# fabrizio-m/TyPLONK

Hardware: AMD Instinct MI355X
Metric: msm_g1_adds_per_s (higher is better)
Workload: dtype u32; 1 GPU; 2^20-term BLS12-381 G1 MSM (KZG commit of a 2^20-row polynomial), SRS [s^i]G with s=2, 1048579 points; window_bits=20, windows=13, parallelism=single GPU, fixed_base_tables=c=20, 13 tables per rank

## Files before the change

### typlonk_amd/csrc/harness/device_reduce_rows.hip

```cpp
#include "../msm_reduce.hip"

#include <algorithm>

using namespace ty;

namespace {

struct Bufs {
    void* p[8] = {};
    int used = 0;
    hipError_t err = hipSuccess;
    uint32_t* zeros(uint64_t points) {
        void* d = nullptr;
        const size_t bytes = (size_t)std::max<uint64_t>(points, 1) * 192;
        if (err == hipSuccess) err = hipMalloc(&d, bytes);
        if (err == hipSuccess) p[used++] = d;
        if (err == hipSuccess) err = hipMemset(d, 0, bytes);
        return static_cast<uint32_t*>(d);
    }
    ~Bufs() {
        for (int i = 0; i < used; ++i) (void)hipFree(p[i]);
    }
};

bool shape_ok(const RcShape& sh) {
    if (sh.nsets < 1 || sh.nsets > 32 || sh.c1 != sh.cl + sh.ch || sh.c1 > 19) return false;
    if (sh.cl < 6 || sh.ch < 6 || sh.cl > 12 || sh.ch > 12 || sh.lhc > sh.ch || sh.llc > sh.cl) return false;
    if (sh.cl - sh.llc > 7 || sh.ch - sh.lhc > 7) return false;
    for (uint32_t set = 0; set < sh.nsets; ++set) {
        uint32_t nbr, nbc, shift;
        rc_bits(sh, set, &nbr, &nbc, &shift);
        if (nbr > RC_NB || nbc > RC_NB) return false;
    }
    return true;
}

__global__ __launch_bounds__(256) void add_pairs_kernel(const uint32_t* __restrict__ a, const uint32_t* __restrict__ b, uint32_t npairs,
                                                        uint32_t* rows_out, uint32_t* lane_out, uint32_t* slow) {
    __shared__ uint32_t buf[4][3][FQR_POINT_WORDS];
    const uint32_t wave = threadIdx.x >> 6, lane = threadIdx.x & 63u, w = blockIdx.x * 4 + wave;
    if (w >= npairs) return;
    const uint32_t c = lane >> 4, i = lane & 15u;
    buf[wave][0][lane] = fqr_limb_of_words(a + (uint64_t)w * 48 + c * 12, i);
    buf[wave][1][lane] = fqr_limb_of_words(b + (uint64_t)w * 48 + c * 12, i);
    __builtin_amdgcn_fence(__ATOMIC_RELEASE, "wavefront");
    __builtin_amdgcn_wave_barrier();
    __builtin_amdgcn_fence(__ATOMIC_ACQUIRE, "wavefront");
    const bool s = g1_add_rows<RowsDev>(buf[wave][0], buf[wave][1], buf[wave][2]);
    __builtin_amdgcn_fence(__ATOMIC_RELEASE, "wavefront");
    __builtin_amdgcn_wave_barrier();
    __builtin_amdgcn_fence(__ATOMIC_ACQUIRE, "wavefront");
    fqr_store_rows<RowsDev>(rows_out + (uint64_t)w * 48, buf[wave][2][lane]);
    if (lane == 0) {
        slow[w] = s ? 1u : 0u;
        st_xyzz(lane_out, w, g1_add(ld_xyzz(a, w), ld_xyzz(b, w)));
    }
}

}

extern "C" int drr_add_pairs(const uint32_t* a, const uint32_t* b, uint32_t npairs, uint32_t* rows_out, uint32_t* lane_out,
                             uint32_t* slow) {
    if (npairs < 1 || npairs > 4096) return (int)hipErrorInvalidValue;
    Bufs m;
    uint32_t* d_a = m.zeros(npairs);
    uint32_t* d_b = m.zeros(npairs);
    uint32_t* d_r = m.zeros(npairs);
    uint32_t* d_l = m.zeros(npairs);
    uint32_t* d_s = m.zeros((npairs + 47) / 48);
    if (m.err == hipSuccess) m.err = hipMemcpy(d_a, a, (size_t)npairs * 192, hipMemcpyHostToDevice);
    if (m.err == hipSuccess) m.err = hipMemcpy(d_b, b, (size_t)npairs * 192, hipMemcpyHostToDevice);
    if (m.err == hipSuccess) {
        hipLaunchKernelGGL(add_pairs_kernel, dim3((npairs + 3) / 4), dim3(256), 0, 0, d_a, d_b, npairs, d_r, d_l, d_s);
        m.err = hipGetLastError();
    }
    if (m.err == hipSuccess) m.err = hipDeviceSynchronize();
    if (m.err == hipSuccess) m.err = hipMemcpy(rows_out, d_r, (size_t)npairs * 192, hipMemcpyDeviceToHost);
    if (m.err == hipSuccess) m.err = hipMemcpy(lane_out, d_l, (size_t)npairs * 192, hipMemcpyDeviceToHost);
    if (m.err == hipSuccess) m.err = hipMemcpy(slow, d_s, (size_t)npairs * 4, hipMemcpyDeviceToHost);
    return (int)m.err;
}

extern "C" int drr_reduce(int form, const uint32_t* shape, const uint32_t* buckets, uint32_t* planes) {
    RcShape sh;
    sh.nsets = shape[0];
    sh.c1 = shape[1];
    sh.ch = shape[2];
    sh.cl = shape[3];
    sh.lhc = shape[4];
    sh.llc = shape[5];
    sh.top_v = shape[6];
    if ((form != 0 && form != 1) || !shape_ok(sh) || !msm_rows_ok(sh)) return (int)hipErrorInvalidValue;
    const uint64_t nb = (uint64_t)sh.nsets << sh.c1;
    const uint64_t nrow = (uint64_t)sh.nsets << (sh.c1 - sh.llc), ncol = (uint64_t)sh.nsets << (sh.c1 - sh.lhc);
    const uint64_t nplanes = (uint64_t)sh.nsets * 2 * RC_NB;
    Bufs m;
    uint32_t* d_buckets = m.zeros(nb);
    uint32_t* part_b = m.zeros(nrow);
    uint32_t* part_a = m.zeros(ncol);
    uint32_t* sums = m.zeros(((uint64_t)sh.nsets << sh.ch) + ((uint64_t)sh.nsets << sh.cl));
    uint32_t* bitsum = m.zeros(nplanes * 64);
    uint32_t* d_planes = m.zeros(nplanes);
    if (m.err == hipSuccess) m.err = hipMemcpy(d_buckets, buckets, (size_t)nb * 192, hipMemcpyHostToDevice);
    if (m.err == hipSuccess) {
        launch_msm_rc_reduce_form(d_buckets, sh, part_b, part_a, sums, bitsum, d_planes, form == 0, 0);
        m.err = hipGetLastError();
    }
    if (m.err == hipSuccess) m.err = hipDeviceSynchronize();
    if (m.err == hipSuccess) m.err = hipMemcpy(planes, d_planes, (size_t)nplanes * 192, hipMemcpyDeviceToHost);
    return (int)m.err;
}
```

### typlonk_amd/csrc/launch.hpp

```cpp
#pragma once
#include <hip/hip_runtime.h>
#include <stdint.h>
#include "ff.hpp"
#include "msm_plan.hpp"
#include "ntt_args.hpp"

namespace ty {

constexpr int PT_WORDS = 32;
constexpr int MSM_HEAVY_GRID = 1024;

struct QuotientArgs {
    const Fr* wires[3];
    const Fr* z;
    const Fr* sel[5];
    const Fr* sigma[3];
    const Fr* pi;
    const Fr* l0;
    const Fr* w_lo;
    const Fr* bx_hi;
    Fr* out;
    uint64_t n4;
    uint32_t w_h;
    uint32_t k0_is_one;
    Fr alpha, alpha2, beta, gamma;
    Fr k[3];
    Fr zh_inv[4];
};
void launch_fr_fill(Fr* out, uint64_t n, const Fr& value, hipStream_t s);
void launch_fr_scale(const Fr* in, uint64_t n, const Fr& factor, Fr* out, hipStream_t s);
void launch_quotient_pointwise(const QuotientArgs& a, hipStream_t s);

struct GrandProductArgs {
    const Fr* wires[3];
    const Fr* sigma[3];
    const Fr* w_lo;
    const Fr* w_hi;
    Fr* num;
    Fr* den;
    uint64_t n;
    uint32_t w_h;
    Fr beta, gamma;
    Fr kbeta[3];
};
void launch_gp_terms(const GrandProductArgs& a, hipStream_t s);
void launch_product_scan(const Fr* in, uint64_t n, int reverse, Fr* block_scratch, Fr* out, hipStream_t s);
void launch_fr_inv(const Fr* in, Fr* out, hipStream_t s);
void launch_gp_finish(const Fr* nprefix, const Fr* dsuffix, const Fr* inv_total , uint64_t n, Fr* z, hipStream_t s);

void launch_open(const Fr* c, uint64_t m, const Fr& z, Fr* q, Fr* blocks, Fr* y, hipStream_t s);
struct LincombArgs {
    const Fr* poly[12];
    Fr scalar[12];
    Fr constant;
    Fr* out;
    uint64_t n;
    uint32_t terms;
};
void launch_lincomb(const LincombArgs& a, hipStream_t s);
void launch_open_multi(const Fr* const* polys, Fr* const* quotients, Fr* const* ys, const uint8_t* zsel, uint32_t count,
                       uint64_t m, const Fr& z0, const Fr& z1, Fr* blocks, hipStream_t s);

bool ntt_big_tiles_available();
void launch_ntt_pass(const NttPassArgs& a, unsigned blocks, unsigned threads, size_t lds_bytes, hipStream_t s);
void launch_ntt_pass30(const NttPassArgs& a, unsigned blocks, unsigned threads, size_t lds_bytes, hipStream_t s);
void launch_ntt_full_table(const Fr* lo, const Fr* hi, uint32_t h, uint64_t S, uint64_t n, Fr* out, hipStream_t s);

void launch_convert_points(uint32_t* pts, const uint8_t* inf, uint64_t n, hipStream_t s);
void launch_msm_digits(const Fr* scalars, uint64_t m, uint32_t c, uint32_t W, uint32_t top_v, uint32_t* keys,
                       uint32_t* counts, hipStream_t s);
void launch_scan(const uint32_t* counts, uint64_t n, uint32_t* block_sums, uint32_t* offsets, uint32_t* cursor,
                 hipStream_t s);
struct MsmSortPtrs {
    uint32_t *blk_hist, *blk_base, *scan_scratch, *blk_cnt, *seg_start, *entries, *counts, *offsets, *sorted, *hist514, *heavy, *tasks,
        *order;
};
void launch_msm_segsort(const Fr* scalars, uint64_t m, const MsmShape& sh, const MsmSortPtrs& p, uint32_t cap, int staged_mode,
                        hipStream_t s);
size_t srs_tables_scratch_bytes(uint64_t len, uint32_t T);
void launch_srs_tables(uint32_t* pts, uint32_t* zbuf, uint64_t len, uint32_t c, uint32_t T, hipStream_t s);
void launch_bucket_order(const uint32_t* counts, const uint32_t* offsets, uint32_t n, uint32_t cap, uint32_t* hist514,
                         uint32_t* order, uint32_t* heavy, uint32_t* tasks, hipStream_t s);
void launch_msm_heavy(const uint32_t* points, const uint32_t* sorted, const uint32_t* hist516, uint32_t* heavy,
                      const uint32_t* tasks, uint32_t* partial, uint32_t* buckets, hipStream_t s);
void launch_msm_scatter(const uint32_t* keys, uint64_t m, uint64_t total, uint32_t* cursor, uint32_t* sorted,
                        hipStream_t s);
void launch_msm_accum(const uint32_t* points, const uint32_t* offsets, const uint32_t* sorted, const uint32_t* order,
                      uint32_t nbuckets, uint32_t cap, bool init, uint32_t lanes, uint32_t split, uint32_t* buckets,
                      hipStream_t s);

void launch_msm_rc_reduce(const uint32_t* buckets, const RcShape& sh, uint32_t* pb, uint32_t* pa, uint32_t* sums,
                          uint32_t* bitsum, uint32_t* out, hipStream_t s);
void launch_msm_rc_reduce_form(const uint32_t* buckets, const RcShape& sh, uint32_t* pb, uint32_t* pa, uint32_t* sums,
                               uint32_t* bitsum, uint32_t* out, bool rows, hipStream_t s);
void launch_msm_rc2_reduce(const uint32_t* buckets, const RcShape& sh, uint32_t* prow, uint32_t* pcol, uint32_t* out,
                           hipStream_t s);
void launch_msm_rc_combine(const uint32_t* planes, const RcShape& sh, uint32_t* set_sums, hipStream_t s);
void launch_fq_inv_selftest(uint64_t seed, uint32_t threads, uint32_t per_thread, uint32_t* out, hipStream_t st);
size_t srs_comb_bytes();
void launch_srs_comb(uint32_t* comb, hipStream_t st);
void launch_srs_generate(const Fr& s, uint64_t start, uint64_t n, const uint32_t* comb, uint32_t* pts, hipStream_t st);
void launch_srs_membership(const uint32_t* pts, uint64_t n, unsigned long long* out, hipStream_t st);
void launch_fr_powers(const Fr& rho, uint64_t n, Fr* pw, Fr* pw_shift, hipStream_t st);
void launch_srs_contribute(const Fr& t, uint64_t n, const uint32_t* src, uint32_t* dst, hipStream_t st);

}
```

### typlonk_amd/csrc/msm_reduce.hip

```cpp
#include "fq30_rows.hpp"
#include "launch.hpp"
#include "msm_common.hpp"

namespace ty {

__global__ __launch_bounds__(64) void msm_rc_partial_kernel(const uint32_t* __restrict__ buckets, RcShape sh,
                                                            uint32_t nrow, uint32_t nrow_pad, uint32_t ncol,
                                                            uint32_t* pb, uint32_t* pa) {
    const uint32_t t = blockIdx.x * 64 + threadIdx.x;
    if (t < nrow_pad) {
        if (t >= nrow) return;
        const uint64_t base = (uint64_t)t << sh.llc;
        G1Xyzz v = ld_xyzz(buckets, base);
        for (uint32_t l = 1; l < (1u << sh.llc); ++l) v = g1_add(v, ld_xyzz(buckets, base + l));
        st_xyzz(pb, t, v);
        return;
    }
    const uint32_t u = t - nrow_pad;
    if (u >= ncol) return;
    const uint32_t per_set = sh.c1 - sh.lhc;
    const uint32_t set = u >> per_set, rem = u & ((1u << per_set) - 1);
    const uint32_t lo = rem & ((1u << sh.cl) - 1), hchunk = rem >> sh.cl;
    const uint64_t first = ((uint64_t)set << sh.c1) + ((uint64_t)(hchunk << sh.lhc) << sh.cl) + lo;
    G1Xyzz v = ld_xyzz(buckets, first);
    for (uint32_t h = 1; h < (1u << sh.lhc); ++h) v = g1_add(v, ld_xyzz(buckets, first + ((uint64_t)h << sh.cl)));
    st_xyzz(pa, ((((uint64_t)set << sh.cl) + lo) << (sh.ch - sh.lhc)) + hchunk, v);
}

struct FoldSeg {
    const uint32_t* in;
    uint32_t* out;
    uint32_t threads, lseq, lanes;
};
__global__ __launch_bounds__(256) void msm_fold_seq_kernel(FoldSeg a, FoldSeg b, uint32_t waves_a, uint32_t waves) {
    const uint32_t wv = blockIdx.x * 4 + (threadIdx.x >> 6);
    if (wv >= waves) return;
    const bool first = wv < waves_a;
    const FoldSeg& g = first ? a : b;
    const uint32_t t = (wv - (first ? 0u : waves_a)) * 64 + (threadIdx.x & 63u);
    G1Xyzz v = G1Xyzz::inf();
    if (t < g.threads) {
        const uint64_t base = (uint64_t)t << g.lseq;
        v = ld_xyzz(g.in, base);
        for (uint32_t i = 1; i < (1u << g.lseq); ++i) v = g1_add(v, ld_xyzz(g.in, base + i));
    }
    v = butterfly_reduce(v, g.lanes);
    if (t < g.threads && (t & (g.lanes - 1)) == 0) st_xyzz(g.out, t / g.lanes, v);
}

__global__ __launch_bounds__(64) void msm_rc_bits_kernel(const uint32_t* __restrict__ sums, RcShape sh, uint32_t rw,
                                                         uint32_t cw, uint32_t* bitsum) {
    const uint32_t nbr_max = sh.ch + 1, nbc_max = sh.cl + 1;
    const uint32_t wps = nbr_max * rw + nbc_max * cw;
    const uint32_t set = blockIdx.x / wps;
    uint32_t r = blockIdx.x % wps, kind = 0, bit, chunk;
    if (r < nbr_max * rw) {
        bit = r / rw;
        chunk = r % rw;
    } else {
        r -= nbr_max * rw;
        kind = 1;
        bit = r / cw;
        chunk = r % cw;
    }
    uint32_t nbr, nbc, shift;
    rc_bits(sh, set, &nbr, &nbc, &shift);
    if (bit >= (kind ? nbc : nbr)) return;
    const uint32_t idx = chunk * 64 + threadIdx.x;
    const uint32_t n_items = kind ? (1u << sh.cl) : (1u << sh.ch);
    G1Xyzz v = G1Xyzz::inf();
    if (idx < n_items && ((rc_weight(sh, set, kind, idx) >> bit) & 1u)) {
        const uint64_t at = kind ? ((uint64_t)sh.nsets << sh.ch) + ((uint64_t)set << sh.cl) + idx : ((uint64_t)set << sh.ch) + idx;
        v = ld_xyzz(sums, at);
    }
    for (uint32_t mask = 1; mask < 64; mask <<= 1) v = butterfly_add(v, (int)mask);
    if (threadIdx.x == 0) st_xyzz(bitsum, (uint64_t)((set * 2 + kind) * RC_NB + bit) * 64 + chunk, v);
}

__global__ __launch_bounds__(64) void msm_rc_final_kernel(const uint32_t* __restrict__ bitsum, RcShape sh, uint32_t rw,
                                                          uint32_t cw, uint32_t* out) {
    const uint32_t bit = blockIdx.x % RC_NB, kind = (blockIdx.x / RC_NB) & 1u, set = blockIdx.x / (2 * RC_NB);
    uint32_t nbr, nbc, shift;
    rc_bits(sh, set, &nbr, &nbc, &shift);
    if (bit >= (kind ? nbc : nbr)) return;
    const uint32_t count = kind ? cw : rw;
    G1Xyzz v = G1Xyzz::inf();
    if (threadIdx.x < count) v = ld_xyzz(bitsum, (uint64_t)blockIdx.x * 64 + threadIdx.x);
    for (uint32_t mask = 1; mask < count; mask <<= 1) v = butterfly_add(v, (int)mask);
    if (threadIdx.x == 0) st_xyzz(out, blockIdx.x, v);
}

__global__ __launch_bounds__(256) void msm_rc2_sums_kernel(const uint32_t* __restrict__ buckets, RcShape sh, uint32_t sr,
                                                           uint32_t sc, uint32_t nwave_row, uint32_t nwave, uint32_t* prow,
                                                           uint32_t* pcol) {
    const uint32_t wv = blockIdx.x * 4 + (threadIdx.x >> 6), lane = threadIdx.x & 63u;
    if (wv >= nwave) return;
    G1Xyzz v;
    if (wv < nwave_row) {
        const uint64_t base = ((uint64_t)wv * 64 + lane) << sr;
        v = ld_xyzz(buckets, base);
        for (uint32_t i = 1; i < (1u << sr); ++i) v = g1_add(v, ld_xyzz(buckets, base + i));
    } else {
        const uint32_t u = wv - nwave_row;
        const uint32_t lpc = sh.ch - 6 - sc;
        const uint32_t rchunk = u & ((1u << lpc) - 1), col = u >> lpc;
        const uint32_t set = col >> sh.cl, lo = col & ((1u << sh.cl) - 1);
        const uint32_t row0 = ((rchunk * 64 + lane) << sc);
        const uint64_t first = ((uint64_t)set << sh.c1) + ((uint64_t)row0 << sh.cl) + lo;
        v = ld_xyzz(buckets, first);
        for (uint32_t i = 1; i < (1u << sc); ++i) v = g1_add(v, ld_xyzz(buckets, first + ((uint64_t)i << sh.cl)));
    }
    v = butterfly_reduce(v, 64);
    if (lane == 0) {
        if (wv < nwave_row) st_xyzz(prow, wv, v);
        else st_xyzz(pcol, wv - nwave_row, v);
    }
}

constexpr int RC2_THREADS = 256;
__global__ __launch_bounds__(RC2_THREADS) void msm_rc2_planes_kernel(const uint32_t* __restrict__ prow,
                                                                     const uint32_t* __restrict__ pcol, RcShape sh,
                                                                     uint32_t lpr, uint32_t lpc, uint32_t* out) {
    __shared__ uint32_t xch[RC2_THREADS / 64][52];
    const uint32_t bit = blockIdx.x % RC_NB, kind = (blockIdx.x / RC_NB) & 1u, set = blockIdx.x / (2 * RC_NB);
    uint32_t nbr, nbc, shift;
    rc_bits(sh, set, &nbr, &nbc, &shift);
    if (bit >= (kind ? nbc : nbr)) return;
    const uint32_t litems = kind ? sh.cl : sh.ch, lp = kind ? lpc : lpr;
    const uint32_t* src = kind ? pcol : prow;
    const uint32_t np = 1u << (litems + lp);
    const uint64_t sbase = (uint64_t)set << (litems + lp);
    G1Xyzz v = G1Xyzz::inf();
    if (rc_set_v(sh, set) == 0) {
        const bool top = kind && bit == sh.cl;
        const uint32_t nsel = (top ? 1u : (1u << (litems - 1))) << lp;
        for (uint32_t idx = threadIdx.x; idx < nsel; idx += blockDim.x) {
            const uint32_t j = idx >> lp, part = idx & ((1u << lp) - 1);
            const uint32_t w = top ? (1u << sh.cl) : (((j >> bit) << (bit + 1)) | (1u << bit) | (j & ((1u << bit) - 1)));
            const uint32_t item = w - kind;
            v = g1_add(v, ld_xyzz(src, sbase + ((uint64_t)item << lp) + part));
        }
    } else {
        for (uint32_t idx = threadIdx.x; idx < np; idx += blockDim.x) {
            const uint32_t item = idx >> lp;
            if ((rc_weight(sh, set, kind, item) >> bit) & 1u) v = g1_add(v, ld_xyzz(src, sbase + idx));
        }
    }
    v = butterfly_reduce(v, 64);
    const uint32_t wave = threadIdx.x >> 6, nwaves = blockDim.x >> 6;
    if ((threadIdx.x & 63) == 0) {
#pragma unroll
        for (int i = 0; i < 13; ++i) {
            xch[wave][i] = v.x.v[i];
            xch[wave][13 + i] = v.y.v[i];
            xch[wave][26 + i] = v.zz.v[i];
            xch[wave][39 + i] = v.zzz.v[i];
        }
    }
    __syncthreads();
    if (wave != 0) return;
    v = G1Xyzz::inf();
    if (threadIdx.x < 2 * nwaves) {
        const uint32_t w = threadIdx.x >> 1;
#pragma unroll
        for (int i = 0; i < 13; ++i) {
            v.x.v[i] = xch[w][i];
            v.y.v[i] = xch[w][13 + i];
            v.zz.v[i] = xch[w][26 + i];
            v.zzz.v[i] = xch[w][39 + i];
        }
    }
#pragma unroll 1
    for (int mask = 2; mask < (int)(2 * nwaves); mask <<= 1) v = butterfly_add4(v, mask);
    if (threadIdx.x == 0) st_xyzz(out, blockIdx.x, v);
}

constexpr uint32_t RC2_LOG_WAVES = 10;
void launch_msm_rc2_reduce(const uint32_t* buckets, const RcShape& sh, uint32_t* prow, uint32_t* pcol, uint32_t* out,
                           hipStream_t s) {
    uint32_t lnb = sh.c1;
    for (uint32_t n = sh.nsets; n > 1; n >>= 1) ++lnb;
    const uint32_t want = lnb > 5 + RC2_LOG_WAVES ? lnb - 5 - RC2_LOG_WAVES : 0;
    const uint32_t sr = want < sh.cl - 6 ? want : sh.cl - 6, sc = want < sh.ch - 6 ? want : sh.ch - 6;
    const uint32_t nwave_row = sh.nsets << (sh.c1 - 6 - sr), nwave_col = sh.nsets << (sh.c1 - 6 - sc);
    hipLaunchKernelGGL(msm_rc2_sums_kernel, dim3((nwave_row + nwave_col + 3) / 4), dim3(256), 0, s, buckets, sh, sr, sc, nwave_row,
                       nwave_row + nwave_col, prow, pcol);
    const uint32_t lpr = sh.cl - 6 - sr, lpc = sh.ch - 6 - sc;
    uint32_t np = 1u << ((sh.ch + lpr) > (sh.cl + lpc) ? (sh.ch + lpr) : (sh.cl + lpc));
    if (sh.top_v == 0 && np > 64) np >>= 1;
    const uint32_t threads = np < 64 ? 64u : (np > (uint32_t)RC2_THREADS ? (uint32_t)RC2_THREADS : np);
    hipLaunchKernelGGL(msm_rc2_planes_kernel, dim3(sh.nsets * 2 * RC_NB), dim3(threads), 0, s, prow, pcol, sh, lpr, lpc, out);
}

__global__ __launch_bounds__(64) void msm_rc_combine_kernel(const uint32_t* __restrict__ planes, RcShape sh,
                                                            uint32_t* set_sums) {
    const uint32_t set = blockIdx.x, kind = threadIdx.x / RC_NB, b = threadIdx.x % RC_NB;
    uint32_t nbr, nbc, shift;
    rc_bits(sh, set, &nbr, &nbc, &shift);
    const bool valid = kind < 2 && b < (kind ? nbc : nbr);
    G1Xyzz v = G1Xyzz::inf();
    if (valid) v = ld_xyzz(planes, (uint64_t)(set * 2 + kind) * RC_NB + b);
    const uint32_t e = valid ? b + (kind ? 0u : shift) : 0u;
    const uint32_t emax = max(nbr ? nbr - 1 + shift : 0u, nbc ? nbc - 1 : 0u);
    for (uint32_t i = 0; i < emax; ++i)
        if (i < e) v = g1_dbl(v);
    for (uint32_t mask = 1; mask < 2 * RC_NB; mask <<= 1) v = butterfly_add(v, (int)mask);
    if (threadIdx.x == 0) st_xyzz(set_sums, set, v);
}

void launch_msm_rc_combine(const uint32_t* planes, const RcShape& sh, uint32_t* set_sums, hipStream_t s) {
    hipLaunchKernelGGL(msm_rc_combine_kernel, dim3(sh.nsets), dim3(64), 0, s, planes, sh, set_sums);
}

constexpr uint32_t ROWS_MAX_ITEMS = 64;
constexpr int ROWS_THREADS0 = 256, ROWS_THREADS1 = 512;

struct RowsPlane {
    uint32_t set, kind, bit, v, litems, nsel, ng;
    bool top, live;
};
__device__ __forceinline__ RowsPlane rows_plane(const RcShape& sh, uint32_t plane, uint32_t ln1) {
    RowsPlane p;
    p.bit = plane % RC_NB;
    p.kind = (plane / RC_NB) & 1u;
    p.set = plane / (2 * RC_NB);
    uint32_t nbr, nbc, shift;
    rc_bits(sh, p.set, &nbr, &nbc, &shift);
    p.live = p.bit < (p.kind ? nbc : nbr);
    p.v = rc_set_v(sh, p.set);
    p.litems = p.kind ? sh.cl : sh.ch;
    p.top = p.v == 0 && p.kind && p.bit == sh.cl;
    p.nsel = p.v == 0 ? (p.top ? 1u : 1u << (p.litems - 1)) : 1u << p.litems;
    p.ng = (p.nsel + (1u << ln1) - 1) >> ln1;
    return p;
}
__device__ __forceinline__ const uint32_t* rows_item(const RcShape& sh, const RowsPlane& p, const uint32_t* rsum,
                                                     const uint32_t* csum, uint32_t idx) {
    const uint32_t* src = p.kind ? csum : rsum;
    const uint64_t sbase = (uint64_t)p.set << p.litems;
    if (p.v == 0) {
        const uint32_t w = p.top ? (1u << sh.cl) : (((idx >> p.bit) << (p.bit + 1)) | (1u << p.bit) | (idx & ((1u << p.bit) - 1)));
        return src + (sbase + (w - p.kind)) * 48;
    }
    return ((rc_weight(sh, p.set, p.kind, idx) >> p.bit) & 1u) ? src + (sbase + idx) * 48 : nullptr;
}
__device__ __forceinline__ uint32_t rows_inf_limb(uint32_t c, uint32_t i) {
    uint32_t r = 0;
#pragma unroll
    for (int j = 0; j < 13; ++j) r = (c < 2 && i == (uint32_t)j) ? fq30_one_limb(j) : r;
    return r;
}

template <int STAGE>
__global__ __launch_bounds__(STAGE ? ROWS_THREADS1 : ROWS_THREADS0) void msm_rows_planes_kernel(
    const uint32_t* __restrict__ rsum, const uint32_t* __restrict__ csum, RcShape sh, uint32_t ln1, uint32_t G, uint32_t* part,
    uint32_t* out) {
    __shared__ uint32_t buf0[ROWS_MAX_ITEMS * FQR_POINT_WORDS];
    __shared__ uint32_t buf1[ROWS_MAX_ITEMS / 2 * FQR_POINT_WORDS];
    const uint32_t plane = STAGE ? blockIdx.x : blockIdx.x / G, g = STAGE ? 0u : blockIdx.x % G;
    const RowsPlane p = rows_plane(sh, plane, ln1);
    if (!p.live || g >= p.ng) return;
    const uint32_t first = g << ln1;
    const uint32_t valid = STAGE ? p.ng : min(1u << ln1, p.nsel - first);
    uint32_t n = 1;
    while (n < valid) n <<= 1;
    for (uint32_t e = threadIdx.x; e < n * FQR_POINT_WORDS; e += blockDim.x) {
        const uint32_t k = e >> 6, c = (e >> 4) & 3u, i = e & 15u;
        const uint32_t* src = nullptr;
        if (k < valid) src = STAGE ? part + ((uint64_t)plane * 64 + k) * 48 : rows_item(sh, p, rsum, csum, first + k);
        buf0[e] = src ? fqr_limb_of_words(src + c * 12, i) : rows_inf_limb(c, i);
    }
    const uint32_t wave = threadIdx.x >> 6, nwaves = blockDim.x >> 6;
    uint32_t* cur = buf0;
    uint32_t* nxt = buf1;
#pragma unroll 1
    for (uint32_t cnt = n; cnt > 1; cnt >>= 1) {
        __syncthreads();
#pragma unroll 1
        for (uint32_t a = wave; a < cnt / 2; a += nwaves)
            g1_add_rows<RowsDev>(cur + (2 * a) * FQR_POINT_WORDS, cur + (2 * a + 1) * FQR_POINT_WORDS, nxt + a * FQR_POINT_WORDS);
        uint32_t* t = cur;
        cur = nxt;
        nxt = t;
    }
    __syncthreads();
    uint32_t* dst = STAGE ? out + (uint64_t)plane * 48 : part + ((uint64_t)plane * 64 + g) * 48;
    if (wave == 0) fqr_store_rows<RowsDev>(dst, cur[threadIdx.x]);
}

static bool msm_rows_ok(const RcShape& sh) {
    const uint32_t lmax = sh.ch > sh.cl ? sh.ch : sh.cl;
    return sh.ch >= 6 && sh.cl >= 6 && lmax - (sh.top_v == 0 ? 1u : 0u) <= 12;
}

void launch_msm_rc_reduce_form(const uint32_t* buckets, const RcShape& sh, uint32_t* pb, uint32_t* pa, uint32_t* sums,
                               uint32_t* bitsum, uint32_t* out, bool rows, hipStream_t s) {
    const uint32_t nrow = sh.nsets << (sh.c1 - sh.llc), ncol = sh.nsets << (sh.c1 - sh.lhc);
    const uint32_t nrow_pad = (nrow + 63) & ~63u;
    hipLaunchKernelGGL(msm_rc_partial_kernel, dim3((nrow_pad + ncol + 63) / 64), dim3(64), 0, s, buckets, sh, nrow, nrow_pad,
                       ncol, pb, pa);
    auto seg = [](const uint32_t* in, uint32_t* out, uint32_t n_in, uint32_t lcnt) {
        FoldSeg g;
        g.in = in;
        g.out = out;
        g.lseq = lcnt < 1 ? lcnt : 1;
        g.lanes = 1u << (lcnt - g.lseq);
        g.threads = n_in >> g.lseq;
        return g;
    };
    uint32_t* rsum = sums;
    uint32_t* csum = sums + ((uint64_t)sh.nsets << sh.ch) * 48;
    const FoldSeg a = seg(pb, rsum, nrow, sh.cl - sh.llc), b = seg(pa, csum, ncol, sh.ch - sh.lhc);
    const uint32_t ba = (a.threads + 63) / 64, bb = (b.threads + 63) / 64;
    hipLaunchKernelGGL(msm_fold_seq_kernel, dim3((ba + bb + 3) / 4), dim3(256), 0, s, a, b, ba, ba + bb);
    if (rows && msm_rows_ok(sh)) {
        const uint32_t lmax = (sh.ch > sh.cl ? sh.ch : sh.cl) - (sh.top_v == 0 ? 1u : 0u);
        const uint32_t ln1 = lmax > 10 ? lmax - 6 : 4;
        const uint32_t G = lmax > ln1 ? 1u << (lmax - ln1) : 1u;
        const uint32_t nplanes = sh.nsets * 2 * RC_NB;
        hipLaunchKernelGGL(msm_rows_planes_kernel<0>, dim3(nplanes * G), dim3(ROWS_THREADS0), 0, s, rsum, csum, sh, ln1, G, bitsum, out);
        hipLaunchKernelGGL(msm_rows_planes_kernel<1>, dim3(nplanes), dim3(ROWS_THREADS1), 0, s, rsum, csum, sh, ln1, G, bitsum, out);
        return;
    }
    if (sh.ch >= 6 && sh.cl >= 6) {
        uint32_t np = 1u << (sh.ch > sh.cl ? sh.ch : sh.cl);
        if (sh.top_v == 0 && np > 64) np >>= 1;
        const uint32_t threads = np < 64 ? 64u : (np > (uint32_t)RC2_THREADS ? (uint32_t)RC2_THREADS : np);
        hipLaunchKernelGGL(msm_rc2_planes_kernel, dim3(sh.nsets * 2 * RC_NB), dim3(threads), 0, s, rsum, csum, sh, 0u, 0u, out);
        return;
    }
    const uint32_t rw = ((1u << sh.ch) + 63) / 64, cw = ((1u << sh.cl) + 63) / 64;
    const uint32_t wps = (sh.ch + 1) * rw + (sh.cl + 1) * cw;
    hipLaunchKernelGGL(msm_rc_bits_kernel, dim3(sh.nsets * wps), dim3(64), 0, s, sums, sh, rw, cw, bitsum);
    hipLaunchKernelGGL(msm_rc_final_kernel, dim3(sh.nsets * 2 * RC_NB), dim3(64), 0, s, bitsum, sh, rw, cw, out);
}

void launch_msm_rc_reduce(const uint32_t* buckets, const RcShape& sh, uint32_t* pb, uint32_t* pa, uint32_t* sums,
                          uint32_t* bitsum, uint32_t* out, hipStream_t s) {
    launch_msm_rc_reduce_form(buckets, sh, pb, pa, sums, bitsum, out, true, s);
}

}
```

Before: 6.882 billion G1-adds/s.

## Share block prefix sums across bit planes in rows reduction; tail fold in LDS

Adds a shared rows-plane mode that is now the default. For sets with top_v==0, a set of block-sum workgroups computes partial sums once, and higher bit planes reuse them instead of re-adding every selected item per plane. The fold kernel stops its lane butterfly at 16 lanes and finishes in LDS with row-parallel adds, and the partial kernel moves to 256-thread blocks. This aims to cut redundant G1 additions in the bucket-reduction phase, at the cost of more complex indexing and more launch geometry to get right.

Result: no change. 6.935 billion G1-adds/s, median of 6 (+0.8%).

```diff
diff --git a/typlonk_amd/csrc/harness/device_reduce_rows.hip b/typlonk_amd/csrc/harness/device_reduce_rows.hip
--- a/typlonk_amd/csrc/harness/device_reduce_rows.hip
+++ b/typlonk_amd/csrc/harness/device_reduce_rows.hip
@@ -81,7 +81,7 @@
     return (int)m.err;
 }
 
-extern "C" int drr_reduce(int form, const uint32_t* shape, const uint32_t* buckets, uint32_t* planes) {
+static int reduce_planes(bool form_ok, RcPlanes form, const uint32_t* shape, const uint32_t* buckets, uint32_t* planes) {
     RcShape sh;
     sh.nsets = shape[0];
     sh.c1 = shape[1];
@@ -90,7 +90,7 @@
     sh.lhc = shape[4];
     sh.llc = shape[5];
     sh.top_v = shape[6];
-    if ((form != 0 && form != 1) || !shape_ok(sh) || !msm_rows_ok(sh)) return (int)hipErrorInvalidValue;
+    if (!form_ok || !shape_ok(sh) || !msm_rows_ok(sh)) return (int)hipErrorInvalidValue;
     const uint64_t nb = (uint64_t)sh.nsets << sh.c1;
     const uint64_t nrow = (uint64_t)sh.nsets << (sh.c1 - sh.llc), ncol = (uint64_t)sh.nsets << (sh.c1 - sh.lhc);
     const uint64_t nplanes = (uint64_t)sh.nsets * 2 * RC_NB;
@@ -103,10 +103,41 @@
     uint32_t* d_planes = m.zeros(nplanes);
     if (m.err == hipSuccess) m.err = hipMemcpy(d_buckets, buckets, (size_t)nb * 192, hipMemcpyHostToDevice);
     if (m.err == hipSuccess) {
-        launch_msm_rc_reduce_form(d_buckets, sh, part_b, part_a, sums, bitsum, d_planes, form == 0, 0);
+        launch_msm_rc_reduce_form(d_buckets, sh, part_b, part_a, sums, bitsum, d_planes, form, 0);
         m.err = hipGetLastError();
     }
     if (m.err == hipSuccess) m.err = hipDeviceSynchronize();
     if (m.err == hipSuccess) m.err = hipMemcpy(planes, d_planes, (size_t)nplanes * 192, hipMemcpyDeviceToHost);
     return (int)m.err;
 }
+
+extern "C" int drr_reduce(int form, const uint32_t* shape, const uint32_t* buckets, uint32_t* planes) {
+    return reduce_planes(form == 0 || form == 1, form == 0 ? RC_PLANES_SHARED : RC_PLANES_LANES, shape, buckets, planes);
+}
+
+extern "C" int drr_reduce_planes(int form, const uint32_t* shape, const uint32_t* buckets, uint32_t* planes) {
+    return reduce_planes(form >= 0 && form <= 2, (RcPlanes)form, shape, buckets, planes);
+}
+
+extern "C" int drr_shared_geometry(const uint32_t* shape, uint32_t* wgs, uint32_t* adds) {
+    RcShape sh;
+    sh.nsets = shape[0];
+    sh.c1 = shape[1];
+    sh.ch = shape[2];
+    sh.cl = shape[3];
+    sh.lhc = shape[4];
+    sh.llc = shape[5];
+    sh.top_v = shape[6];
+    if (!shape_ok(sh) || !msm_rows_ok(sh) || sh.top_v != 0) return (int)hipErrorInvalidValue;
+    const RowsGeom gm = rows_geom(sh, true);
+    if (!gm.shared) return (int)hipErrorInvalidValue;
+    *wgs = *adds = 0;
+    for (uint32_t kind = 0; kind < 2; ++kind) {
+        const uint32_t l = kind ? sh.cl : sh.ch;
+        const uint32_t nsel = rows_sel_planes(gm, l) * rows_sel_groups(gm, l), nblk = 1u << (l - gm.lb);
+        const uint32_t per_group = std::min(1u << gm.ln1, 1u << (l - 1));
+        *wgs += sh.nsets * (nsel + nblk);
+        *adds += sh.nsets * (nsel * (per_group - 1) + nblk * ((1u << gm.lb) - 1));
+    }
+    return 0;
+}
diff --git a/typlonk_amd/csrc/launch.hpp b/typlonk_amd/csrc/launch.hpp
--- a/typlonk_amd/csrc/launch.hpp
+++ b/typlonk_amd/csrc/launch.hpp
@@ -91,8 +91,9 @@
 
 void launch_msm_rc_reduce(const uint32_t* buckets, const RcShape& sh, uint32_t* pb, uint32_t* pa, uint32_t* sums,
                           uint32_t* bitsum, uint32_t* out, hipStream_t s);
+enum RcPlanes { RC_PLANES_LANES = 0, RC_PLANES_ROWS = 1, RC_PLANES_SHARED = 2 };
 void launch_msm_rc_reduce_form(const uint32_t* buckets, const RcShape& sh, uint32_t* pb, uint32_t* pa, uint32_t* sums,
-                               uint32_t* bitsum, uint32_t* out, bool rows, hipStream_t s);
+                               uint32_t* bitsum, uint32_t* out, RcPlanes form, hipStream_t s);
 void launch_msm_rc2_reduce(const uint32_t* buckets, const RcShape& sh, uint32_t* prow, uint32_t* pcol, uint32_t* out,
                            hipStream_t s);
 void launch_msm_rc_combine(const uint32_t* planes, const RcShape& sh, uint32_t* set_sums, hipStream_t s);
diff --git a/typlonk_amd/csrc/msm_reduce.hip b/typlonk_amd/csrc/msm_reduce.hip
--- a/typlonk_amd/csrc/msm_reduce.hip
+++ b/typlonk_amd/csrc/msm_reduce.hip
@@ -4,10 +4,11 @@
 
 namespace ty {
 
-__global__ __launch_bounds__(64) void msm_rc_partial_kernel(const uint32_t* __restrict__ buckets, RcShape sh,
-                                                            uint32_t nrow, uint32_t nrow_pad, uint32_t ncol,
-                                                            uint32_t* pb, uint32_t* pa) {
-    const uint32_t t = blockIdx.x * 64 + threadIdx.x;
+constexpr uint32_t RC_PARTIAL_THREADS = 256;
+__global__ __launch_bounds__(RC_PARTIAL_THREADS) void msm_rc_partial_kernel(const uint32_t* __restrict__ buckets, RcShape sh,
+                                                                            uint32_t nrow, uint32_t nrow_pad, uint32_t ncol,
+                                                                            uint32_t* pb, uint32_t* pa) {
+    const uint32_t t = blockIdx.x * RC_PARTIAL_THREADS + threadIdx.x;
     if (t < nrow_pad) {
         if (t >= nrow) return;
         const uint64_t base = (uint64_t)t << sh.llc;
@@ -31,7 +32,10 @@
     const uint32_t* in;
     uint32_t* out;
     uint32_t threads, lseq, lanes;
+    uint32_t sub;
 };
+constexpr uint32_t FOLD_SUB = 16;
+constexpr uint32_t FOLD_TAIL_POINTS = 64 / FOLD_SUB;
 __global__ __launch_bounds__(256) void msm_fold_seq_kernel(FoldSeg a, FoldSeg b, uint32_t waves_a, uint32_t waves) {
     const uint32_t wv = blockIdx.x * 4 + (threadIdx.x >> 6);
     if (wv >= waves) return;
@@ -44,8 +48,49 @@
         v = ld_xyzz(g.in, base);
         for (uint32_t i = 1; i < (1u << g.lseq); ++i) v = g1_add(v, ld_xyzz(g.in, base + i));
     }
-    v = butterfly_reduce(v, g.lanes);
-    if (t < g.threads && (t & (g.lanes - 1)) == 0) st_xyzz(g.out, t / g.lanes, v);
+    if (g.sub == g.lanes) {
+        v = butterfly_reduce(v, g.lanes);
+        if (t < g.threads && (t & (g.lanes - 1)) == 0) st_xyzz(g.out, t / g.lanes, v);
+        return;
+    }
+    __shared__ uint32_t tl[4][(FOLD_TAIL_POINTS + FOLD_TAIL_POINTS / 2) * FQR_POINT_WORDS];
+    const uint32_t sub = g.sub;
+    v = butterfly_reduce(v, sub);
+    const uint32_t lane = threadIdx.x & 63u;
+    uint32_t* cur = tl[threadIdx.x >> 6];
+    uint32_t* nxt = cur + FOLD_TAIL_POINTS * FQR_POINT_WORDS;
+    if ((lane & (sub - 1)) == 0) {
+        uint32_t* pt = cur + (lane / sub) * FQR_POINT_WORDS;
+#pragma unroll
+        for (int i = 0; i < 13; ++i) {
+            pt[i] = v.x.v[i];
+            pt[16 + i] = v.y.v[i];
+            pt[32 + i] = v.zz.v[i];
+            pt[48 + i] = v.zzz.v[i];
+        }
+#pragma unroll
+        for (int i = 13; i < 16; ++i) pt[i] = pt[16 + i] = pt[32 + i] = pt[48 + i] = 0u;
+    }
+    const uint32_t nout = 64 / g.lanes;
+#pragma unroll 1
+    for (uint32_t cnt = 64 / sub; cnt > nout; cnt >>= 1) {
+        __builtin_amdgcn_fence(__ATOMIC_RELEASE, "wavefront");
+        __builtin_amdgcn_wave_barrier();
+        __builtin_amdgcn_fence(__ATOMIC_ACQUIRE, "wavefront");
+#pragma unroll 1
+        for (uint32_t a = 0; a < cnt / 2; ++a)
+            g1_add_rows<RowsDev>(cur + (2 * a) * FQR_POINT_WORDS, cur + (2 * a + 1) * FQR_POINT_WORDS, nxt + a * FQR_POINT_WORDS);
+        uint32_t* x = cur;
+        cur = nxt;
+        nxt = x;
+    }
+    __builtin_amdgcn_fence(__ATOMIC_RELEASE, "wavefront");
+    __builtin_amdgcn_wave_barrier();
+    __builtin_amdgcn_fence(__ATOMIC_ACQUIRE, "wavefront");
+    const uint32_t t0 = t - lane;
+#pragma unroll 1
+    for (uint32_t j = 0; j < nout; ++j)
+        if (t0 + j * g.lanes < g.threads) fqr_store_rows<RowsDev>(g.out + (uint64_t)(t0 / g.lanes + j) * 48, cur[j * FQR_POINT_WORDS + lane]);
 }
 
 __global__ __launch_bounds__(64) void msm_rc_bits_kernel(const uint32_t* __restrict__ sums, RcShape sh, uint32_t rw,
@@ -251,23 +296,99 @@
     return r;
 }
 
+constexpr uint32_t ROWS_FOLD_BLOCKS = 32;
+
+struct RowsGeom {
+    uint32_t ln1, G;
+    uint32_t lb;
+    uint32_t W;
+    bool shared;
+};
+TY_HD uint32_t rows_sel_planes(const RowsGeom& gm, uint32_t litems) {
+    return (1u << (litems - gm.lb)) > ROWS_FOLD_BLOCKS ? gm.lb : gm.lb - 1;
+}
+TY_HD uint32_t rows_sel_groups(const RowsGeom& gm, uint32_t litems) {
+    return ((1u << (litems - 1)) + (1u << gm.ln1) - 1) >> gm.ln1;
+}
+TY_HD uint32_t rows_kind_wgs(const RowsGeom& gm, uint32_t litems) {
+    return rows_sel_planes(gm, litems) * rows_sel_groups(gm, litems) + (1u << (litems - gm.lb));
+}
+TY_HD RowsGeom rows_geom(const RcShape& sh, bool share) {
+    RowsGeom gm;
+    const uint32_t lkind = sh.ch > sh.cl ? sh.ch : sh.cl;
+    const uint32_t lmax = lkind - (sh.top_v == 0 ? 1u : 0u);
+    gm.ln1 = lmax > 10 ? lmax - 6 : 4;
+    gm.G = lmax > gm.ln1 ? 1u << (lmax - gm.ln1) : 1u;
+    gm.lb = lkind > 10 ? lkind - 6 : 4;
+    gm.shared = share && gm.lb <= 6;
+    gm.W = 2 * RC_NB * gm.G;
+    if (gm.shared) {
+        const uint32_t w = rows_kind_wgs(gm, sh.ch) + rows_kind_wgs(gm, sh.cl);
+        gm.W = (sh.top_v != 0 && gm.W > w) ? gm.W : w;
+    }
+    return gm;
+}
+
 template <int STAGE>
 __global__ __launch_bounds__(STAGE ? ROWS_THREADS1 : ROWS_THREADS0) void msm_rows_planes_kernel(
-    const uint32_t* __restrict__ rsum, const uint32_t* __restrict__ csum, RcShape sh, uint32_t ln1, uint32_t G, uint32_t* part,
+    const uint32_t* __restrict__ rsum, const uint32_t* __restrict__ csum, RcShape sh, RowsGeom gm, uint32_t* part,
     uint32_t* out) {
     __shared__ uint32_t buf0[ROWS_MAX_ITEMS * FQR_POINT_WORDS];
     __shared__ uint32_t buf1[ROWS_MAX_ITEMS / 2 * FQR_POINT_WORDS];
-    const uint32_t plane = STAGE ? blockIdx.x : blockIdx.x / G, g = STAGE ? 0u : blockIdx.x % G;
-    const RowsPlane p = rows_plane(sh, plane, ln1);
-    if (!p.live || g >= p.ng) return;
-    const uint32_t first = g << ln1;
-    const uint32_t valid = STAGE ? p.ng : min(1u << ln1, p.nsel - first);
+    const uint32_t set = STAGE ? blockIdx.x / (2 * RC_NB) : blockIdx.x / gm.W;
+    const bool shared = gm.shared && rc_set_v(sh, set) == 0;
+    uint32_t plane = blockIdx.x, g = 0;
+    bool block = false;
+    if (!STAGE) {
+        uint32_t r = blockIdx.x % gm.W;
+        if (!shared) {
+            if (r >= 2 * RC_NB * gm.G) return;
+            plane = set * 2 * RC_NB + r / gm.G;
+            g = r % gm.G;
+        } else {
+            uint32_t kind = 0;
+            if (r >= rows_kind_wgs(gm, sh.ch)) {
+                r -= rows_kind_wgs(gm, sh.ch);
+                kind = 1;
+            }
+            const uint32_t litems = kind ? sh.cl : sh.ch;
+            if (r >= rows_kind_wgs(gm, litems)) return;
+            const uint32_t ngs = rows_sel_groups(gm, litems), nsel_wgs = rows_sel_planes(gm, litems) * ngs;
+            block = r >= nsel_wgs;
+            g = block ? r - nsel_wgs : r % ngs;
+            plane = (set * 2 + kind) * RC_NB + (block ? gm.lb : r / ngs);
+        }
+    }
+    const RowsPlane p = rows_plane(sh, plane, gm.ln1);
+    if (!block && (!p.live || g >= p.ng)) return;
+    const uint32_t nblk = 1u << (p.litems - (shared ? gm.lb : 0u));
+    const bool fold = shared && nblk <= ROWS_FOLD_BLOCKS;
+    const uint32_t first = g << gm.ln1;
+    uint32_t valid;
+    if (!STAGE) valid = block ? 1u << gm.lb : min(1u << gm.ln1, p.nsel - first);
+    else if (!shared) valid = p.ng;
+    else if (p.top) valid = 1;
+    else if (p.bit >= gm.lb) valid = nblk / 2;
+    else valid = (fold && p.bit == gm.lb - 1) ? nblk : p.ng;
     uint32_t n = 1;
     while (n < valid) n <<= 1;
     for (uint32_t e = threadIdx.x; e < n * FQR_POINT_WORDS; e += blockDim.x) {
         const uint32_t k = e >> 6, c = (e >> 4) & 3u, i = e & 15u;
         const uint32_t* src = nullptr;
-        if (k < valid) src = STAGE ? part + ((uint64_t)plane * 64 + k) * 48 : rows_item(sh, p, rsum, csum, first + k);
+        if (k < valid) {
+            if (!STAGE && block) {
+                const uint32_t w = (g << gm.lb) + k;
+                if (w >= p.kind) src = (p.kind ? csum : rsum) + (((uint64_t)p.set << p.litems) + (w - p.kind)) * 48;
+            } else if (!STAGE || (shared && p.top)) {
+                src = rows_item(sh, p, rsum, csum, first + k);
+            } else if (shared && p.bit >= gm.lb) {
+                const uint32_t t = p.bit - gm.lb;
+                const uint32_t gs = ((k >> t) << (t + 1)) | (1u << t) | (k & ((1u << t) - 1));
+                src = part + ((uint64_t)(plane - t) * 64 + gs) * 48;
+            } else {
+                src = part + ((uint64_t)plane * 64 + k) * 48;
+            }
+        }
         buf0[e] = src ? fqr_limb_of_words(src + c * 12, i) : rows_inf_limb(c, i);
     }
     const uint32_t wave = threadIdx.x >> 6, nwaves = blockDim.x >> 6;
@@ -276,6 +397,8 @@
 #pragma unroll 1
     for (uint32_t cnt = n; cnt > 1; cnt >>= 1) {
         __syncthreads();
+        if (!STAGE && block && fold && cnt == 2 && wave == 1)
+            fqr_store_rows<RowsDev>(part + ((uint64_t)(plane - 1) * 64 + g) * 48, cur[FQR_POINT_WORDS + (threadIdx.x & 63u)]);
 #pragma unroll 1
         for (uint32_t a = wave; a < cnt / 2; a += nwaves)
             g1_add_rows<RowsDev>(cur + (2 * a) * FQR_POINT_WORDS, cur + (2 * a + 1) * FQR_POINT_WORDS, nxt + a * FQR_POINT_WORDS);
@@ -294,18 +417,20 @@
 }
 
 void launch_msm_rc_reduce_form(const uint32_t* buckets, const RcShape& sh, uint32_t* pb, uint32_t* pa, uint32_t* sums,
-                               uint32_t* bitsum, uint32_t* out, bool rows, hipStream_t s) {
+                               uint32_t* bitsum, uint32_t* out, RcPlanes form, hipStream_t s) {
     const uint32_t nrow = sh.nsets << (sh.c1 - sh.llc), ncol = sh.nsets << (sh.c1 - sh.lhc);
-    const uint32_t nrow_pad = (nrow + 63) & ~63u;
-    hipLaunchKernelGGL(msm_rc_partial_kernel, dim3((nrow_pad + ncol + 63) / 64), dim3(64), 0, s, buckets, sh, nrow, nrow_pad,
-                       ncol, pb, pa);
-    auto seg = [](const uint32_t* in, uint32_t* out, uint32_t n_in, uint32_t lcnt) {
+    const uint32_t nrow_pad = (nrow + RC_PARTIAL_THREADS - 1) & ~(RC_PARTIAL_THREADS - 1);
+    hipLaunchKernelGGL(msm_rc_partial_kernel, dim3((nrow_pad + ncol + RC_PARTIAL_THREADS - 1) / RC_PARTIAL_THREADS),
+                       dim3(RC_PARTIAL_THREADS), 0, s, buckets, sh, nrow, nrow_pad, ncol, pb, pa);
+    const bool tail = form != RC_PLANES_LANES && msm_rows_ok(sh);
+    auto seg = [tail](const uint32_t* in, uint32_t* out, uint32_t n_in, uint32_t lcnt) {
         FoldSeg g;
         g.in = in;
         g.out = out;
         g.lseq = lcnt < 1 ? lcnt : 1;
         g.lanes = 1u << (lcnt - g.lseq);
         g.threads = n_in >> g.lseq;
+        g.sub = (tail && g.lanes > FOLD_SUB) ? FOLD_SUB : g.lanes;
         return g;
     };
     uint32_t* rsum = sums;
@@ -313,13 +438,11 @@
     const FoldSeg a = seg(pb, rsum, nrow, sh.cl - sh.llc), b = seg(pa, csum, ncol, sh.ch - sh.lhc);
     const uint32_t ba = (a.threads + 63) / 64, bb = (b.threads + 63) / 64;
     hipLaunchKernelGGL(msm_fold_seq_kernel, dim3((ba + bb + 3) / 4), dim3(256), 0, s, a, b, ba, ba + bb);
-    if (rows && msm_rows_ok(sh)) {
-        const uint32_t lmax = (sh.ch > sh.cl ? sh.ch : sh.cl) - (sh.top_v == 0 ? 1u : 0u);
-        const uint32_t ln1 = lmax > 10 ? lmax - 6 : 4;
-        const uint32_t G = lmax > ln1 ? 1u << (lmax - ln1) : 1u;
+    if (form != RC_PLANES_LANES && msm_rows_ok(sh)) {
+        const RowsGeom gm = rows_geom(sh, form == RC_PLANES_SHARED);
         const uint32_t nplanes = sh.nsets * 2 * RC_NB;
-        hipLaunchKernelGGL(msm_rows_planes_kernel<0>, dim3(nplanes * G), dim3(ROWS_THREADS0), 0, s, rsum, csum, sh, ln1, G, bitsum, out);
-        hipLaunchKernelGGL(msm_rows_planes_kernel<1>, dim3(nplanes), dim3(ROWS_THREADS1), 0, s, rsum, csum, sh, ln1, G, bitsum, out);
+        hipLaunchKernelGGL(msm_rows_planes_kernel<0>, dim3(sh.nsets * gm.W), dim3(ROWS_THREADS0), 0, s, rsum, csum, sh, gm, bitsum, out);
+        hipLaunchKernelGGL(msm_rows_planes_kernel<1>, dim3(nplanes), dim3(ROWS_THREADS1), 0, s, rsum, csum, sh, gm, bitsum, out);
         return;
     }
     if (sh.ch >= 6 && sh.cl >= 6) {
@@ -337,7 +460,7 @@
 
 void launch_msm_rc_reduce(const uint32_t* buckets, const RcShape& sh, uint32_t* pb, uint32_t* pa, uint32_t* sums,
                           uint32_t* bitsum, uint32_t* out, hipStream_t s) {
-    launch_msm_rc_reduce_form(buckets, sh, pb, pa, sums, bitsum, out, true, s);
-}
-
-}
+    launch_msm_rc_reduce_form(buckets, sh, pb, pa, sums, bitsum, out, RC_PLANES_SHARED, s);
+}
+
+}
```
